# Sukikui/PTI-LDM-VAE

Hardware: AMD Instinct MI355X
Metric: vae_train_images_per_sec_256x256 (higher is better)
Workload: dtype fp16 forward operands + activations / bf16 backward operands + gradients, fp32 accumulate; 1 GPU; config/vae_dente_no_adv.json 256x256x1 batch 32/GPU: fwd + L1 + 1e-3*KL + bwd + all-reduce + Adam (perceptual term omitted: --perceptual times it; adversarial branch inactive before epoch 6, --adv times it); global_batch=32, parallelism=dp1

## Files before the change

pti_ldm_vae_amd/csrc/conv_common.h:

```cpp
#pragma once
#include "pti_common.h"

namespace pti_conv {

struct ConvArgs {
  const bf16* x;
  const unsigned char* w;
  const float* bias;
  const stat_t* in_stats;
  const float* gamma;
  const float* beta;
  const bf16* res;
  bf16* y;
  stat_t* out_stats;
  int N, H, W, Cin, Ho, Wo, Cout;
  int mode, prologue, groups, out_groups;
  float eps, inv_cnt;
  int tiles_x, tiles_y;
  int gn_mode;
  int g_groups;
  float g_inv_cnt, g_eps;
  const stat_t* g_stats; const float* g_gamma; const float* g_beta;
  float* g_sums;
  int g_T;
  bf16* act_out;
  int in_f16, res_f16, out_f16;
  int pool2;
  int relu_out;
  int w_f16;
  const bf16* x2;
  const float* p_sums;
  int x2_f16;
};
constexpr int PRO_GNB = 3;

typedef _Float16 f16x8 __attribute__((ext_vector_type(8)));
template <bool OPH>
__device__ __forceinline__ f32x16 mfma32(const bf16x8& a, const bf16x8& b, const f32x16& c) {
  if constexpr (OPH)
    return __builtin_amdgcn_mfma_f32_32x32x16_f16(__builtin_bit_cast(f16x8, a), __builtin_bit_cast(f16x8, b), c, 0, 0, 0);
  else
    return __builtin_amdgcn_mfma_f32_32x32x16_bf16(a, b, c, 0, 0, 0);
}

__host__ __device__ constexpr int pick_ck2(int cin, int ct) {
  const int ck = cin % 128 == 0 ? 128 : (cin % 64 == 0 ? 64 : 32);
  const int cap = ct >= 128 ? 128 : (ct == 64 ? 64 : 32);
  return ck < cap ? ck : cap;
}

template <int NV, int N, int O>
__device__ __forceinline__ void fold32_level(float (&v)[NV], int j) {
  if constexpr (O >= 1) {
    if constexpr (N > 1) {
      const bool hi = (j & O) != 0;
#pragma unroll
      for (int i = 0; i < N / 2; ++i) {
        const float send = hi ? v[i] : v[i + N / 2];
        const float keep = hi ? v[i + N / 2] : v[i];
        v[i] = keep + __shfl_xor(send, O, 64);
      }
    } else {
      v[0] += __shfl_xor(v[0], O, 64);
    }
    fold32_level<NV, (N > 1 ? N / 2 : 1), O / 2>(v, j);
  }
}
template <int NV>
__device__ __forceinline__ void fold32(float (&v)[NV], int j) { fold32_level<NV, NV, 16>(v, j); }

template <int KS, int CK, int CT, int PXF>
struct Cfg2 {
  static constexpr int WN = CT / 32, WM = 4 / WN;
  static constexpr int TH2 = 2 * PXF * WM, TW2 = 16;
  static constexpr int HH = TH2 + KS - 1, HW = TW2 + KS - 1;
  static constexpr int NP = HH * HW;
  static constexpr int NC = CK / 8;
  static constexpr int PIXB = CK * 2;
  static constexpr int NT = CT / 32;
  static constexpr int KPC = CK / 16;
  static constexpr int KBC = KS * KS * KPC;
  static constexpr int R = (KS == 3) ? (PXF == 2 ? 3 : 9) : KBC;
  static constexpr int WGS_PER_CU = PXF == 2 ? 4 : 2;
  static constexpr int HALO_BYTES = NP * PIXB;
  static constexpr int KEY_SHIFT = (NC == 16) ? 0 : (NC == 8 ? 1 : 2);
  static constexpr int HITERS = (NP * NC + 255) / 256;
  static constexpr int MPX = 32 * PXF * WM;
  static constexpr int EPITCH = CT * 2 + 16;
  static constexpr int EPI_BYTES = MPX * EPITCH;
  static constexpr int ENC = CT / 8;
  static constexpr int EITERS = MPX * ENC / 256;
  static constexpr int STAT_OFF = HALO_BYTES > EPI_BYTES ? HALO_BYTES : EPI_BYTES;
  static constexpr int RT_OFF = STAT_OFF + 1024 + 256;
  static constexpr int RT_BYTES = MPX * CT * 2;
  static constexpr int BIAS_OFF = RT_OFF + RT_BYTES;
  static constexpr bool GT_IN_TAIL = HALO_BYTES - EPI_BYTES >= 8 * CT;
  static constexpr int GT_OFF = GT_IN_TAIL ? EPI_BYTES : BIAS_OFF + 4 * CT;
  static constexpr int LDS_BYTES = BIAS_OFF + 4 * CT + (GT_IN_TAIL ? 0 : 8 * CT);
};


int launch_conv_ws128(const ConvArgs& a, hipStream_t st);

}
```

pti_ldm_vae_amd/csrc/conv_mfma.hip:

```cpp
#include "conv_common.h"

namespace {
using namespace pti_conv;

constexpr int TH = 8, TW = 16;

__host__ __device__ constexpr int pick_cout_tile(int cout) { return cout % 128 == 0 ? 128 : (cout % 64 == 0 ? 64 : 32); }
__host__ __device__ constexpr int pick_ck(int cin, int stride2) {
  int ck = cin % 128 == 0 ? 128 : (cin % 64 == 0 ? 64 : 32);
  return (stride2 && ck > 64) ? 64 : ck;
}
__host__ __device__ constexpr int pick_wblk(int kbc, int nt) {
  int best = 1;
  for (int w = 1; w <= kbc; ++w)
    if (kbc % w == 0 && w * nt <= 16) best = w;
  return best;
}

template <int KS, int S, int CK, int COUT_TILE>
struct Cfg {
  static constexpr int HH = (TH - 1) * S + KS, HW = (TW - 1) * S + KS;
  static constexpr int NP = HH * HW;
  static constexpr int NC = CK / 8;
  static constexpr int PIXB = CK * 2;
  static constexpr int NT = COUT_TILE / 32;
  static constexpr int KPC = CK / 16;
  static constexpr int KBC = KS * KS * KPC;
  static constexpr int WBLK = pick_wblk(KBC, NT);
  static constexpr int NSTEP = KBC / WBLK;
  static constexpr int STEPB = WBLK * NT * 1024;
  static constexpr int WM = (NT >= 2) ? 2 : 4, WN = 4 / WM;
  static constexpr int PXF = 4 / WM;
  static constexpr int CF = NT / WN;
  static constexpr int HALO_BYTES = NP * PIXB;
  static constexpr int LDS_BYTES = HALO_BYTES + 2 * STEPB;
  static constexpr int KEY_SHIFT = (NC == 16) ? 0 : (NC == 8 ? 1 : 2);
  static constexpr int WPIECES = (STEPB / 16 + 255) / 256;
  static constexpr int HITERS = (NP * NC + 255) / 256;
};

template <int KS, int S, int CK, int COUT_TILE, bool OPH>
__global__ __launch_bounds__(256, 2) void conv_mfma_kernel(ConvArgs a) {
  if (a.out_f16) fp16_saturate_on();
  using C = Cfg<KS, S, CK, COUT_TILE>;
  __shared__ __attribute__((aligned(16))) unsigned char smem[C::LDS_BYTES];
  unsigned char* halo = smem;
  unsigned char* wbuf = smem + C::HALO_BYTES;

  const int tid = threadIdx.x, lane = tid & 63, wave = tid >> 6;
  const int hsel = lane >> 5;
  int t = blockIdx.x;
  const int tile_x = t % a.tiles_x;
  t /= a.tiles_x;
  const int tile_y = t % a.tiles_y;
  const int n = t / a.tiles_y;
  const int oy0 = tile_y * TH, ox0 = tile_x * TW;
  const int ct = blockIdx.y;
  const int nchunks = a.Cin / CK;
  const int wm = wave / C::WN, wn = wave % C::WN;

  const int pad_lo = (a.mode == PTI_CONV_S2PAD) ? 0 : (a.mode == PTI_CONV_ZINS ? 2 : (KS - 1) / 2);
  const int vy0 = oy0 * S - pad_lo, vx0 = ox0 * S - pad_lo;
  const bool twox = (a.mode == PTI_CONV_UP2) || (a.mode == PTI_CONV_ZINS);
  const int VH = twox ? 2 * a.H : a.H, VW = twox ? 2 * a.W : a.W;

  int pbase[C::PXF][KS];
  int tkey[KS];
  {
    const int j = lane & 31;
    const int tx = j & 15;
#pragma unroll
    for (int kw = 0; kw < KS; ++kw) {
      const int hx = tx * S + kw;
      tkey[kw] = (hsel ^ ((hx >> C::KEY_SHIFT) & (C::NC - 1))) << 4;
#pragma unroll
      for (int i = 0; i < C::PXF; ++i) {
        const int ty = 2 * (wm * C::PXF + i) + (j >> 4);
        pbase[i][kw] = ((ty * S) * C::HW + hx) * C::PIXB;
      }
    }
  }

// ... 124 lines not shown
  const int j = lane & 31;
  stat_t* sstat = reinterpret_cast<stat_t*>(smem);
  const bool do_stats = a.out_stats != nullptr;
  const int ocpg = do_stats ? a.Cout / a.out_groups : 1;
  if (do_stats) {
    if (tid < 2 * a.out_groups) sstat[tid] = 0;
    __syncthreads();
  }
#pragma unroll
  for (int i = 0; i < C::PXF; ++i) {
    const int ty = 2 * (wm * C::PXF + i) + (j >> 4), tx = j & 15;
    const int oy = oy0 + ty, ox = ox0 + tx;
    const bool inb = (oy < a.Ho) && (ox < a.Wo);
    const size_t pix = ((size_t)(n * a.Ho + oy) * a.Wo + ox) * a.Cout;
#pragma unroll
    for (int c = 0; c < C::CF; ++c) {
#pragma unroll
      for (int q = 0; q < 4; ++q) {
        const int co = ct * COUT_TILE + (wn * C::CF + c) * 32 + 8 * q + 4 * hsel;
        float v0 = acc[i][c][4 * q + 0], v1 = acc[i][c][4 * q + 1], v2 = acc[i][c][4 * q + 2],
              v3 = acc[i][c][4 * q + 3];
        if (a.bias) {
          const f32x4 b = *(const f32x4*)(a.bias + co);
          v0 += b[0]; v1 += b[1]; v2 += b[2]; v3 += b[3];
        }
        u32x2 packed = u32x2{0u, 0u};
        if (inb) {
          if (a.res) {
            const u32x2 rr = *(const u32x2*)(a.res + pix + co);
            float e0, e1, e2, e3;
            unpack2f(rr[0], a.res_f16, e0, e1);
            unpack2f(rr[1], a.res_f16, e2, e3);
            v0 += e0; v1 += e1; v2 += e2; v3 += e3;
          }
          packed = pack4f(v0, v1, v2, v3, a.out_f16);
          *(u32x2*)(a.y + pix + co) = packed;
        }
        if (do_stats) {
          float r0, r1, r2, r3;
          unpack2f(packed[0], a.out_f16, r0, r1);
          unpack2f(packed[1], a.out_f16, r2, r3);
          if (!inb) r0 = r1 = r2 = r3 = 0.f;
          if (ocpg >= 4) {
            float s1 = (r0 + r1) + (r2 + r3), s2 = (r0 * r0 + r1 * r1) + (r2 * r2 + r3 * r3);
#pragma unroll
            for (int o = 16; o > 0; o >>= 1) {
              s1 += __shfl_xor(s1, o, 64);
              s2 += __shfl_xor(s2, o, 64);
            }
            if (j == 0) {
              const int g = co / ocpg;
              stat_add(&sstat[2 * g], s1);
              stat_add(&sstat[2 * g + 1], s2);
            }
          } else {
            float a1 = r0 + r1, a2 = r0 * r0 + r1 * r1, b1 = r2 + r3, b2 = r2 * r2 + r3 * r3;
#pragma unroll
            for (int o = 16; o > 0; o >>= 1) {
              a1 += __shfl_xor(a1, o, 64);
              a2 += __shfl_xor(a2, o, 64);
              b1 += __shfl_xor(b1, o, 64);
              b2 += __shfl_xor(b2, o, 64);
            }
            if (j == 0) {
              const int g = co / 2;
              stat_add(&sstat[2 * g], a1);
              stat_add(&sstat[2 * g + 1], a2);
              stat_add(&sstat[2 * g + 2], b1);
              stat_add(&sstat[2 * g + 3], b2);
            }
          }
        }
      }
    }
  }
  if (do_stats) {
    __syncthreads();
    const int g0 = (ct * COUT_TILE) / ocpg, ng = COUT_TILE / ocpg;
    if (tid < 2 * ng)
      atomicAdd((unsigned long long*)&a.out_stats[(n * a.out_groups + g0) * 2 + tid], (unsigned long long)sstat[2 * g0 + tid]);
  }
}

template <int KS, int CK, int CT, int PXF, bool SAVE, int FM, int PRO>
__global__ __launch_bounds__(256, (PXF == 2 ? 4 : 2)) void conv_mfma2_kernel(ConvArgs a) {
  using C = Cfg2<KS, CK, CT, PXF>;
  const int prologue = PRO >= 0 ? PRO : a.prologue;
  const bool gn_on = FM == 3 ? true : (FM == 0 ? a.gn_mode != 0 : false);
  const bool in_f16 = FM == 0 ? (bool)a.in_f16 : (FM == 1);
  const bool res_f16 = FM == 0 ? (bool)a.res_f16 : (FM == 1 || FM == 3);
  const bool out_f16 = FM == 0 ? (bool)a.out_f16 : (FM == 1);
  constexpr bool OPH = (FM == 1);
  if (out_f16) fp16_saturate_on();
  __shared__ __attribute__((aligned(16))) unsigned char smem[C::LDS_BYTES];
  unsigned char* halo = smem;
  const int tid = threadIdx.x, lane = tid & 63, wave = tid >> 6;
  const int hsel = lane >> 5;
  int t = blockIdx.x;
  const int tile_x = t % a.tiles_x;
  t /= a.tiles_x;
  const int tile_y = t % a.tiles_y;
  const int n = t / a.tiles_y;
  const int oy0 = tile_y * C::TH2, ox0 = tile_x * C::TW2;
  const int ct = blockIdx.y;
  const int nchunks = a.Cin / CK;
  const int wm = wave / C::WN, wn = wave % C::WN;

  const int pad_lo = (a.mode == PTI_CONV_ZINS) ? 2 : (KS - 1) / 2;
  const int vy0 = oy0 - pad_lo, vx0 = ox0 - pad_lo;
  const bool twox = (a.mode == PTI_CONV_UP2) || (a.mode == PTI_CONV_ZINS);
  const int VH = twox ? 2 * a.H : a.H, VW = twox ? 2 * a.W : a.W;

  int pbase[KS], tkey[KS];
  {
    const int j = lane & 31, tx = j & 15, row0 = 2 * PXF * wm + (j >> 4);
#pragma unroll
    for (int kw = 0; kw < KS; ++kw) {
      const int hx = tx + kw;
      tkey[kw] = (hsel ^ ((hx >> C::KEY_SHIFT) & (C::NC - 1))) << 4;
      pbase[kw] = (row0 * C::HW + hx) * C::PIXB;
    }
  }
  f32x16 acc[PXF];
#pragma unroll
  for (int i = 0; i < PXF; ++i)
#pragma unroll
    for (int r = 0; r < 16; ++r) acc[i][r] = 0.f;

  const int lc = tid % C::NC, lp0 = tid / C::NC;
  constexpr int PSTEP = 256 / C::NC;
  const int cpg = a.Cin / (a.groups > 0 ? a.groups : 1);
  reinterpret_cast<float*>(smem + C::STAT_OFF)[tid] = 0.f;
  float* sfl = reinterpret_cast<float*>(smem + C::STAT_OFF + 1024);
  if (prologue == PTI_PRO_GN || prologue == PTI_PRO_GN_SILU) {
    if (tid < 2 * a.groups) sfl[tid] = stat_f(a.in_stats, n * a.groups * 2 + tid);
  } else if (gn_on) {
    if (tid < 2 * a.g_groups) sfl[tid] = stat_f(a.g_stats, n * a.g_groups * 2 + tid);
  }
  float gq = 0.f, bq = 0.f;
  if (gn_on) {
    if (tid < CT) {
      gq = a.g_gamma[ct * CT + tid];
      bq = a.g_beta[ct * CT + tid];
    }
  } else if (a.bias) {
    if (tid < CT) reinterpret_cast<float*>(smem + C::BIAS_OFF)[tid] = a.bias[ct * CT + tid];
  }
  if (a.res) {
#pragma unroll
    for (int it = 0; it < C::EITERS; ++it) {
      const int slot = it * 256 + tid;
      const int p = slot / C::ENC, c = slot % C::ENC;
      const int oy = oy0 + p / C::TW2, ox = ox0 + p % C::TW2;
      if (oy < a.Ho && ox < a.Wo) {
        const bf16* src = a.res + ((size_t)(n * a.Ho + oy) * a.Wo + ox) * a.Cout + ct * CT + ((c ^ ((p >> 2) & (C::ENC - 1))) << 3);
        __builtin_amdgcn_global_load_lds((const __attribute__((address_space(1))) void*)src,
                                         (__attribute__((address_space(3))) void*)(smem + C::RT_OFF + (it * 256 + wave * 64) * 16),
                                         16, 0, 0);
      }
    }
  }

  const int epc = tid % C::ENC, epp0 = tid / C::ENC;
  constexpr int EPSTEP = 256 / C::ENC;

  for (int chunk = 0; chunk < nchunks; ++chunk) {
    const unsigned char* wlane =
        a.w + ((size_t)(ct * nchunks + chunk) * C::KBC * C::NT + wn) * 1024 + lane * 16;
    bf16x8 wa[C::R], wb[C::R];
    auto wload = [&](bf16x8 (&dst)[C::R], int g) {
#pragma unroll
      for (int u = 0; u < C::R; ++u) {
        int kb = g * C::R + u;
        kb = kb < C::KBC ? kb : C::KBC - 1;
        dst[u] = *(const bf16x8*)(wlane + (size_t)kb * C::NT * 1024);
      }
    };
    constexpr bool WLATE = (SAVE && PXF == 2) || PRO == PRO_GNB;
    if constexpr (!WLATE) wload(wa, 0);

    u32x4 raw[C::HITERS];
    u32x4 raw2[PRO == PRO_GNB ? C::HITERS : 1];
    bool ok[C::HITERS];
    {
      const __amdgpu_buffer_rsrc_t xrs = __builtin_amdgcn_make_buffer_rsrc(
          const_cast<bf16*>(a.x), 0, (unsigned)a.N * (unsigned)a.H * (unsigned)a.W * (unsigned)a.Cin * 2u, 0x00020000);
      const __amdgpu_buffer_rsrc_t x2rs = __builtin_amdgcn_make_buffer_rsrc(
          const_cast<bf16*>(PRO == PRO_GNB ? a.x2 : a.x), 0, (unsigned)a.N * (unsigned)a.H * (unsigned)a.W * (unsigned)a.Cin * 2u, 0x00020000);
      const unsigned base = ((unsigned)n * a.H * a.W * a.Cin + chunk * CK + lc * 8) * 2u;
      const unsigned rowb = (unsigned)a.W * a.Cin * 2u, pixb = (unsigned)a.Cin * 2u;
#pragma unroll
      for (int it = 0; it < C::HITERS; ++it) {
        const int p = lp0 + it * PSTEP;
        const int hy = p / C::HW, hx = p - hy * C::HW;
        const int vy = vy0 + hy, vx = vx0 + hx;
        bool v = (p < C::NP) && (unsigned)vy < (unsigned)VH && (unsigned)vx < (unsigned)VW;
        int iy = vy, ix = vx;
        if (twox) {
          if (a.mode == PTI_CONV_ZINS) v = v && !((vy | vx) & 1);
          iy = vy >> 1;
          ix = vx >> 1;
        }
        ok[it] = v;
        const unsigned off = v ? base + (unsigned)iy * rowb + (unsigned)ix * pixb : 0x80000000u;
        raw[it] = __builtin_bit_cast(u32x4, __builtin_amdgcn_raw_buffer_load_b128(xrs, off, 0, 0));
        if constexpr (PRO == PRO_GNB) raw2[it] = __builtin_bit_cast(u32x4, __builtin_amdgcn_raw_buffer_load_b128(x2rs, off, 0, 0));
      }
    }
    if (chunk == 0) __syncthreads();
    float sc[8], sh[8];
    [[maybe_unused]] float gnb_b = 0.f, gnb_d = 0.f;
    if constexpr (PRO == PRO_GNB) {
      const int ch0 = chunk * CK + lc * 8, g = ch0 / cpg;
      const float mean = stat_f(a.in_stats, (n * a.groups + g) * 2) * a.inv_cnt;
      const float rstd = rsqrtf(fmaxf(stat_f(a.in_stats, (n * a.groups + g) * 2 + 1) * a.inv_cnt - mean * mean, 0.f) + a.eps);
      float t1 = 0.f, t2 = 0.f;
      for (int cc = g * cpg; cc < (g + 1) * cpg; ++cc) {
        const f32x2 sv = *(const f32x2*)(a.p_sums + ((size_t)n * a.Cin + cc) * 2);
        const float gm = a.gamma[cc];
        t1 += gm * sv[0];
        t2 += gm * sv[1];
      }
      const float c1 = t1 * a.inv_cnt, c2 = t2 * a.inv_cnt;
#pragma unroll
      for (int j = 0; j < 8; ++j) sc[j] = rstd * a.gamma[ch0 + j];
      gnb_b = -rstd * rstd * c2;
      gnb_d = -rstd * c1 - gnb_b * mean;
    } else if (prologue != PTI_PRO_NONE) {
      float mu_[8], rs_[8];
      gn_params<8>(sfl, a.gamma, a.beta, chunk * CK + lc * 8, cpg, a.inv_cnt, a.eps, sc, sh, mu_, rs_);
    }
    if (chunk > 0) __syncthreads();
#pragma unroll
    for (int it = 0; it < C::HITERS; ++it) {
      const int p = lp0 + it * PSTEP;
      if (p < C::NP) {
        const int hy = p / C::HW, hx = p - hy * C::HW;
        u32x4 r = raw[it];
        if constexpr (PRO == PRO_GNB) {
          if (ok[it]) {
            float f[8], h[8];
            unpack8(r, f);
            unpack8f(raw2[it], h, a.x2_f16 != 0);
#pragma unroll
            for (int j = 0; j < 8; ++j) f[j] = fmaf(sc[j], f[j], fmaf(gnb_b, h[j], gnb_d));
            r = pack8(f);
          }
        } else if (prologue != PTI_PRO_NONE && ok[it]) {
          float f[8];
          unpack8f(r, f, in_f16);
          if (PXF == 4 && prologue == PTI_PRO_GN_SILU) {
#pragma unroll
            for (int j = 0; j < 8; j += 2) {
              const f32x2 o = gn_silu2(f32x2{f[j], f[j + 1]}, f32x2{sc[j], sc[j + 1]}, f32x2{sh[j], sh[j + 1]});
              f[j] = o[0];
              f[j + 1] = o[1];
            }
          } else {
#pragma unroll
            for (int j = 0; j < 8; ++j) {
              float v = f[j] * sc[j] + sh[j];
              if (prologue == PTI_PRO_GN_SILU) v = silu_f(v);
              f[j] = v;
            }
          }
          r = OPH ? pack8f(f, true) : pack8(f);
        } else if (in_f16 && !OPH) {
          float f[8];
          unpack8f(r, f, true);
          r = pack8(f);
        }
        const int key = (hx >> C::KEY_SHIFT) & (C::NC - 1);
        *(u32x4*)(halo + p * C::PIXB + ((lc ^ key) << 4)) = r;
      }
    }
    __syncthreads();

    if constexpr (SAVE) {
      if (ct == 0) {
        constexpr int PL = (KS - 1) / 2;
        constexpr int SITERS = C::TH2 * C::TW2 * C::NC / 256;
        const __amdgpu_buffer_rsrc_t srs = __builtin_amdgcn_make_buffer_rsrc(
            a.act_out, 0, (unsigned)a.N * (unsigned)a.H * (unsigned)a.W * (unsigned)a.Cin * 2u, 0x00020000);
#pragma unroll 1
        for (int it = 0; it < SITERS; ++it) {
          const int idx = tid + it * 256;
          const int c8 = idx % C::NC, pi = idx / C::NC;
          const int hy = pi / C::TW2 + PL, hx = pi % C::TW2 + PL;
          const int vy = vy0 + hy, vx = vx0 + hx;
          if (vy < a.H && vx < a.W) {
            const int key = (hx >> C::KEY_SHIFT) & (C::NC - 1);
            u32x4 piece = *(const u32x4*)(halo + (hy * C::HW + hx) * C::PIXB + ((c8 ^ key) << 4));
            if constexpr (OPH) {
              float f[8];
              unpack8f(piece, f, true);
              piece = pack8(f);
            }
            __builtin_amdgcn_raw_buffer_store_b128(__builtin_bit_cast(bu32x4, piece), srs,
                                                   ((unsigned)((n * a.H + vy) * a.W + vx) * a.Cin + chunk * CK + c8 * 8) * 2u, 0, 2 );
          }
        }
      }
    }

    if constexpr (WLATE) wload(wa, 0);
    const int txl = lane & 15;
    auto baddr = [&](int kb) -> const unsigned char* {
      kb = kb < C::KBC ? kb : C::KBC - 1;
      const int tap = kb / C::KPC, kc = kb - tap * C::KPC;
      const int kh = (KS == 3) ? tap / 3 : 0, kw = tap - kh * KS;
      const int hx = txl + kw;
      const int tk = (hsel ^ ((hx >> C::KEY_SHIFT) & (C::NC - 1))) << 4;
      return halo + pbase[0] + (kh * C::HW + kw) * C::PIXB + ((kc * 32) ^ tk);
    };
    bf16x8 b0[PXF], b1[PXF];
    auto bread = [&](bf16x8 (&dst)[PXF], int kb) {
      const unsigned char* bp = baddr(kb);
#pragma unroll
      for (int i = 0; i < PXF; ++i) dst[i] = *(const bf16x8*)(bp + 2 * i * C::HW * C::PIXB);
    };
    auto group = [&](const bf16x8 (&w)[C::R], int g) {
      const int kb0 = g * C::R;
#pragma unroll
      for (int u = 0; u < C::R; ++u) {
        if ((u & 1) == 0) {
          bread(b1, kb0 + u + 1);
#pragma unroll
          for (int i = 0; i < PXF; ++i) acc[i] = mfma32<OPH>(w[u], b0[i], acc[i]);
        } else {
          bread(b0, kb0 + u + 1);
#pragma unroll
          for (int i = 0; i < PXF; ++i) acc[i] = mfma32<OPH>(w[u], b1[i], acc[i]);
        }
      }
      if (C::R & 1) {
#pragma unroll
        for (int i = 0; i < PXF; ++i) b0[i] = b1[i];
      }
    };
    constexpr int NG = C::KBC / C::R;
    bread(b0, 0);
    if constexpr (NG == 1) {
      group(wa, 0);
    } else {
#pragma clang loop unroll(disable)
      for (int g = 0; g < NG; g += 2) {
        wload(wb, g + 1);
        group(wa, g);
        wload(wa, g + 2);
        group(wb, g + 1);
      }
    }
  }

  const int j = lane & 31;
  unsigned char* etile = smem;
  const bool do_stats = (FM == 2 || FM == 3) ? false : a.out_stats != nullptr;
  const int ocpg = do_stats ? a.Cout / a.out_groups : 1;
  __syncthreads();
  float* gtab = reinterpret_cast<float*>(smem + C::GT_OFF);
  if (gn_on) {
    if (tid < CT) {
      gtab[tid] = gq;
      gtab[CT + tid] = bq;
    }
    __syncthreads();
  }
  const unsigned char* rtile = smem + C::RT_OFF;
  const int col0 = wn * 32 + 4 * hsel;
  float st1[4] = {0.f, 0.f, 0.f, 0.f}, st2[4] = {0.f, 0.f, 0.f, 0.f};
  float su1[4] = {0.f, 0.f, 0.f, 0.f}, su2[4] = {0.f, 0.f, 0.f, 0.f};
  if (gn_on) {
    const int gcpg = a.Cout / a.g_groups;
    float* gsm = reinterpret_cast<float*>(smem + C::STAT_OFF);
    float L[32];
#pragma unroll
    for (int q = 0; q < 4; ++q) {
      const int col = col0 + 8 * q, ch0 = ct * CT + col;
      float scv[4], shv[4], muv[4], rsv[4], l1[4] = {0.f, 0.f, 0.f, 0.f}, l2[4] = {0.f, 0.f, 0.f, 0.f};
      gn_params<4>(sfl, gtab - ct * CT, gtab + CT - ct * CT, ch0, gcpg, a.g_inv_cnt, a.g_eps, scv, shv, muv, rsv);
      float nmr[4];
#pragma unroll
      for (int r = 0; r < 4; ++r) nmr[r] = -muv[r] * rsv[r];
#pragma unroll
      for (int i = 0; i < PXF; ++i) {
        const int p = (2 * PXF * wm + 2 * i + (j >> 4)) * 16 + (j & 15);
        const bool inb = (oy0 + (p >> 4) < a.Ho) && (ox0 + (p & 15) < a.Wo);
        unsigned char* ep = etile + p * C::EPITCH + col * 2;
        const u32x2 rr = *(const u32x2*)(rtile + p * (CT * 2) + ((((col >> 3) ^ (p >> 2)) & (C::ENC - 1)) << 4) + (col & 7) * 2);
        float xv[4];
        unpack2f(rr[0], res_f16, xv[0], xv[1]);
        unpack2f(rr[1], res_f16, xv[2], xv[3]);
        float dv[4];
#pragma unroll
        for (int r = 0; r < 4; ++r) {
          float v = acc[i][4 * q + r];
          if (a.gn_mode == 2) v *= dsilu_f(xv[r] * scv[r] + shv[r]);
          dv[r] = v;
        }
        const u32x2 packed = pack4(dv[0], dv[1], dv[2], dv[3]);
        *(u32x2*)ep = packed;
        if (inb) {
#pragma unroll
          for (int r = 0; r < 4; ++r) {
            l1[r] += dv[r];
            l2[r] = fmaf(dv[r], fmaf(xv[r], rsv[r], nmr[r]), l2[r]);
          }
        }
      }
#pragma unroll
      for (int r = 0; r < 4; ++r) {
        L[8 * q + 2 * r] = l1[r];
        L[8 * q + 2 * r + 1] = l2[r];
      }
    }
    fold32<32>(L, j);
    gsm[wm * 2 * CT + col0 * 2 + 16 * (j >> 3) + (j & 7)] = L[0];
  } else {
#pragma unroll
  for (int i = 0; i < PXF; ++i) {
    const int p = (2 * PXF * wm + 2 * i + (j >> 4)) * 16 + (j & 15);
    const bool inb = (oy0 + (p >> 4) < a.Ho) && (ox0 + (p & 15) < a.Wo);
#pragma unroll
    for (int q = 0; q < 4; ++q) {
      const int col = col0 + 8 * q;
      float v0 = acc[i][4 * q + 0], v1 = acc[i][4 * q + 1], v2 = acc[i][4 * q + 2], v3 = acc[i][4 * q + 3];
      if (a.bias) {
        const f32x4 b = *(const f32x4*)(smem + C::BIAS_OFF + col * 4);
        v0 += b[0]; v1 += b[1]; v2 += b[2]; v3 += b[3];
      }
      unsigned char* ep = etile + p * C::EPITCH + col * 2;
      if (a.res) {
        const u32x2 rr = *(const u32x2*)(rtile + p * (CT * 2) + ((((col >> 3) ^ (p >> 2)) & (C::ENC - 1)) << 4) + (col & 7) * 2);
        float e0, e1, e2, e3;
        unpack2f(rr[0], res_f16, e0, e1);
        unpack2f(rr[1], res_f16, e2, e3);
        v0 += e0; v1 += e1; v2 += e2; v3 += e3;
      }
      if constexpr (FM == 1 && PRO == PTI_PRO_NONE) {
        if (a.relu_out) { v0 = fmaxf(v0, 0.f); v1 = fmaxf(v1, 0.f); v2 = fmaxf(v2, 0.f); v3 = fmaxf(v3, 0.f); }
      }
      const u32x2 packed = pack4f(v0, v1, v2, v3, out_f16);
      *(u32x2*)ep = packed;
      if (do_stats && inb) {
        float r0, r1, r2, r3;
        unpack2f(packed[0], out_f16, r0, r1);
        unpack2f(packed[1], out_f16, r2, r3);
        if (ocpg >= 4) {
          st1[q] += (r0 + r1) + (r2 + r3);
          st2[q] += (r0 * r0 + r1 * r1) + (r2 * r2 + r3 * r3);
        } else {
          st1[q] += r0 + r1; st2[q] += r0 * r0 + r1 * r1;
          su1[q] += r2 + r3; su2[q] += r2 * r2 + r3 * r3;
        }
      }
    }
  }
  }
  if (do_stats) {
    stat_t* sstat = reinterpret_cast<stat_t*>(smem + C::STAT_OFF);
    if (ocpg >= 4) {
      float v[8];
#pragma unroll
      for (int q = 0; q < 4; ++q) { v[2 * q] = st1[q]; v[2 * q + 1] = st2[q]; }
      fold32<8>(v, j);
      if ((j & 3) == 0) {
        const int idx = j >> 2, q = idx >> 1;
        const int g = (ct * CT + col0 + 8 * q) / ocpg;
        stat_add(&sstat[2 * g + (idx & 1)], v[0]);
      }
    } else {
      float v[16];
#pragma unroll
      for (int q = 0; q < 4; ++q) { v[4 * q] = st1[q]; v[4 * q + 1] = st2[q]; v[4 * q + 2] = su1[q]; v[4 * q + 3] = su2[q]; }
      fold32<16>(v, j);
      if ((j & 1) == 0) {
        const int idx = j >> 1, q = idx >> 2;
        const int g = (ct * CT + col0 + 8 * q) / 2;
        stat_add(&sstat[2 * g + (idx & 3)], v[0]);
      }
    }
  }
  __syncthreads();
  const __amdgpu_buffer_rsrc_t yrs = __builtin_amdgcn_make_buffer_rsrc(
      a.y, 0, ((unsigned)a.N * (unsigned)a.Ho * (unsigned)a.Wo * (unsigned)a.Cout * 2u) >> (a.pool2 ? 2 : 0), 0x00020000);
  if ((FM == 0 || FM == 2) && a.pool2) {
    constexpr int PITERS = (C::EITERS + 3) / 4;
#pragma unroll
    for (int it = 0; it < PITERS; ++it) {
      const int idx = tid + it * 256;
      const int c8 = idx % C::ENC, pp = idx / C::ENC;
      const int py = pp / 8, px = pp % 8;
      const int oy = (oy0 >> 1) + py, ox = (ox0 >> 1) + px;
      if (pp < C::MPX / 4 && oy < (a.Ho >> 1) && ox < (a.Wo >> 1)) {
        const unsigned char* src = etile + ((2 * py) * 16 + 2 * px) * C::EPITCH + c8 * 16;
        float s_[8], f_[8];
        unpack8f(*(const u32x4*)src, s_, out_f16);
        unpack8f(*(const u32x4*)(src + C::EPITCH), f_, out_f16);
#pragma unroll
        for (int q = 0; q < 8; ++q) s_[q] += f_[q];
        unpack8f(*(const u32x4*)(src + 16 * C::EPITCH), f_, out_f16);
#pragma unroll
        for (int q = 0; q < 8; ++q) s_[q] += f_[q];
        unpack8f(*(const u32x4*)(src + 17 * C::EPITCH), f_, out_f16);
#pragma unroll
        for (int q = 0; q < 8; ++q) s_[q] += f_[q];
        __builtin_amdgcn_raw_buffer_store_b128(__builtin_bit_cast(bu32x4, pack8f(s_, out_f16)), yrs,
                                               ((unsigned)((n * (a.Ho >> 1) + oy) * (a.Wo >> 1) + ox) * a.Cout + ct * CT + c8 * 8) * 2u, 0, 2);
      }
    }
  } else
#pragma unroll
  for (int it = 0; it < C::EITERS; ++it) {
    const int p = epp0 + it * EPSTEP;
    const int oy = oy0 + (p >> 4), ox = ox0 + (p & 15);
    if (oy < a.Ho && ox < a.Wo)
      __builtin_amdgcn_raw_buffer_store_b128(__builtin_bit_cast(bu32x4, *(const u32x4*)(etile + p * C::EPITCH + epc * 16)), yrs,
                                             ((unsigned)((n * a.Ho + oy) * a.Wo + ox) * a.Cout + ct * CT + epc * 8) * 2u, 0, 2);
  }
  if (gn_on) {
    if (tid < 2 * CT) {
      const float* gsm = reinterpret_cast<const float*>(smem + C::STAT_OFF);
      float v = gsm[tid];
#pragma unroll
      for (int m = 1; m < C::WM; ++m) v += gsm[m * 2 * CT + tid];
      a.g_sums[(((size_t)n * a.g_T + tile_y * a.tiles_x + tile_x) * a.Cout + ct * CT) * 2 + tid] = v;
    }
  } else if (do_stats) {
    const stat_t* sstat = reinterpret_cast<const stat_t*>(smem + C::STAT_OFF);
    const int g0 = (ct * CT) / ocpg, ng = CT / ocpg;
    if (tid < 2 * ng)
      atomicAdd((unsigned long long*)&a.out_stats[(n * a.out_groups + g0) * 2 + tid], (unsigned long long)sstat[2 * g0 + tid]);
  }
}

template <int KS, int CK, int CT, int PXF>
int launch2_cfg(ConvArgs a, hipStream_t st) {
  using C = Cfg2<KS, CK, CT, PXF>;
  a.tiles_x = cdiv(a.Wo, C::TW2);
  a.tiles_y = cdiv(a.Ho, C::TH2);
  a.g_T = a.tiles_x * a.tiles_y;
  dim3 grid(a.N * a.tiles_x * a.tiles_y, a.Cout / CT);
  const bool res = a.res != nullptr;
  const int fm = (a.w_f16 && a.in_f16 && a.out_f16 && (a.res_f16 || !res)) ? 1
               : (!a.in_f16 && !a.out_f16 && (!a.res_f16 || !res)) ? 2
               : (!a.in_f16 && !a.out_f16 && a.res_f16) ? 3 : 0;
  const bool fwd_silu = fm == 1 && a.prologue == PTI_PRO_GN_SILU && !a.gn_mode && !a.pool2;
  const bool fwd_plain = fm == 1 && a.prologue == PTI_PRO_NONE && !a.gn_mode && !a.pool2;
  const bool dgrad = fm == 2 && a.prologue == PTI_PRO_NONE && !a.gn_mode && !a.out_stats;
  const bool dgrad_gn = fm == 3 && a.prologue == PTI_PRO_NONE && a.gn_mode && !a.out_stats && !a.pool2;
  if (a.x2) {
    if constexpr (KS == 3 && PXF == 4 && CT == 128) {
      if (!(fm == 3 && a.gn_mode && a.act_out && !a.out_stats && !a.pool2 && a.mode == PTI_CONV_S1 && !a.relu_out)) return 4;
      PTI_LAUNCH((conv_mfma2_kernel<KS, CK, CT, PXF, true, 3, PRO_GNB>), grid, dim3(256), 0, st, a);
      return 0;
    } else {
      return 4;
    }
// ... 348 lines not shown
```

Before: 2735 images/s.

## Specialize narrow 3x3 conv kernel with incremental addressing and DPP reductions

For the PXF=2, 3x3, fixed-format conv variants, this adds a NARROW specialization. Halo, residual and saved-activation address generation moves to strength-reduced incremental offsets, and whole waves with no work skip the halo-load iterations. The GroupNorm backward epilogue is rewritten with precomputed per-quad parameters and a pinned dSiLU. The cross-lane stat folds now use DPP, ds_swizzle and permlane16_swap instead of generic shuffles. The aim is to cut integer ALU, LDS-shuffle and register cost in the hot conv kernel, at the cost of more code paths and a possible change in numerical ordering.

```diff
diff --git a/pti_ldm_vae_amd/csrc/conv_common.h b/pti_ldm_vae_amd/csrc/conv_common.h
--- a/pti_ldm_vae_amd/csrc/conv_common.h
+++ b/pti_ldm_vae_amd/csrc/conv_common.h
@@ -69,6 +69,43 @@
 template <int NV>
 __device__ __forceinline__ void fold32(float (&v)[NV], int j) { fold32_level<NV, NV, 16>(v, j); }
 
+template <int O>
+__device__ __forceinline__ float xor_lane(float v) {
+  static_assert(O == 8 || O == 4 || O == 2 || O == 1, "xor distance inside a 16-lane row");
+  const unsigned u = __float_as_uint(v);
+  if constexpr (O == 8) return __uint_as_float(__builtin_amdgcn_update_dpp(0u, u, 0x128 , 0xf, 0xf, false));
+  else if constexpr (O == 4) return __uint_as_float(__builtin_amdgcn_ds_swizzle(u, 0x101f ));
+  else if constexpr (O == 2) return __uint_as_float(__builtin_amdgcn_update_dpp(0u, u, 0x4e , 0xf, 0xf, false));
+  else return __uint_as_float(__builtin_amdgcn_update_dpp(0u, u, 0xb1 , 0xf, 0xf, false));
+}
+template <int NV, int N, int O>
+__device__ __forceinline__ void fold32x_level(float (&v)[NV], int j) {
+  if constexpr (O >= 1) {
+    if constexpr (N > 1 && O == 16) {
+#pragma unroll
+      for (int i = 0; i < N / 2; ++i) {
+        const auto sw = __builtin_amdgcn_permlane16_swap(__float_as_uint(v[i]), __float_as_uint(v[i + N / 2]), false, false);
+        v[i] = __uint_as_float(sw[0]) + __uint_as_float(sw[1]);
+      }
+    } else if constexpr (N > 1) {
+      const bool hi = (j & O) != 0;
+#pragma unroll
+      for (int i = 0; i < N / 2; ++i) {
+        const float send = hi ? v[i] : v[i + N / 2];
+        const float keep = hi ? v[i + N / 2] : v[i];
+        v[i] = keep + xor_lane<O>(send);
+      }
+    } else if constexpr (O == 16) {
+      v[0] += __shfl_xor(v[0], 16, 64);
+    } else {
+      v[0] += xor_lane<O>(v[0]);
+    }
+    fold32x_level<NV, (N > 1 ? N / 2 : 1), O / 2>(v, j);
+  }
+}
+template <int NV>
+__device__ __forceinline__ void fold32x(float (&v)[NV], int j) { fold32x_level<NV, NV, 16>(v, j); }
+
 template <int KS, int CK, int CT, int PXF>
 struct Cfg2 {
   static constexpr int WN = CT / 32, WM = 4 / WN;
diff --git a/pti_ldm_vae_amd/csrc/conv_mfma.hip b/pti_ldm_vae_amd/csrc/conv_mfma.hip
--- a/pti_ldm_vae_amd/csrc/conv_mfma.hip
+++ b/pti_ldm_vae_amd/csrc/conv_mfma.hip
@@ -1,3 +1,5 @@
+#include <type_traits>
+
 #include "conv_common.h"
 
 namespace {
@@ -288,6 +290,78 @@
   }
 }
 
+__device__ __forceinline__ f32x2 dsilu_times2(f32x2 acc, f32x2 v) {
+#pragma clang fp contract(off)
+#pragma clang fp reassociate(off)
+  const f32x2 t = v * -1.4426950408889634f;
+  f32x2 s;
+  s[0] = __builtin_amdgcn_rcpf(1.0f + __builtin_amdgcn_exp2f(t[0]));
+  s[1] = __builtin_amdgcn_rcpf(1.0f + __builtin_amdgcn_exp2f(t[1]));
+  const f32x2 sa = s * acc;
+  f32x2 b = (1.0f - s) * v;
+  asm("" : "+v"(b));
+  return sa * (1.0f + b);
+}
+
+__device__ __forceinline__ void gn_quad_pinned(const float* sfl, const float* gam, const float* bet, int ch0, int cpg,
+                                               float inv_cnt, float eps, float* sc, float* sh, float* rs, float* nmr) {
+#pragma clang fp contract(off)
+#pragma clang fp reassociate(off)
+  const bool pow2 = (cpg & (cpg - 1)) == 0;
+  const f32x4 gm = *(const f32x4*)gam, bt = *(const f32x4*)bet;
+  auto rstd_fused = [&](const f32x2 st, float& mean) {
+    mean = st[0] * inv_cnt;
+    const float t = st[1] * inv_cnt;
+    return __builtin_amdgcn_rsqf(fmaxf(__builtin_fmaf(-mean, mean, t), 0.f) + eps);
+  };
+  if (pow2 && cpg >= 4) {
+    float mean;
+    const float rstd = rstd_fused(*(const f32x2*)(sfl + 2 * (ch0 >> __builtin_ctz(cpg))), mean);
+    const float nm = rstd * -mean;
+#pragma unroll
+    for (int r = 0; r < 4; ++r) {
+      sc[r] = rstd * gm[r];
+      sh[r] = __builtin_fmaf(nm, gm[r], bt[r]);
+      rs[r] = rstd;
+      nmr[r] = nm;
+    }
+  } else if (cpg == 2) {
+#pragma unroll
+    for (int k = 0; k < 2; ++k) {
+      float mean;
+      const float rstd = rstd_fused(*(const f32x2*)(sfl + 2 * ((ch0 >> 1) + k)), mean);
+      const float rm = rstd * mean;
+#pragma unroll
+      for (int r = 2 * k; r < 2 * k + 2; ++r) {
+        sc[r] = rstd * gm[r];
+        sh[r] = __builtin_fmaf(-rm, gm[r], bt[r]);
+        rs[r] = rstd;
+        nmr[r] = -rm;
+      }
+    }
+  } else {
+#pragma unroll
+    for (int r = 0; r < 4; ++r) {
+      const int g = cpg == 1 ? ch0 + r : (ch0 + r) / cpg;
+      const f32x2 st = *(const f32x2*)(sfl + 2 * g);
+      const float mean = st[0] * inv_cnt;
+      float t = st[1] * inv_cnt, var;
+      if (r < 2) {
+        float mm = mean * mean;
+        asm("" : "+v"(t), "+v"(mm));
+        var = t - mm;
+      } else {
+        var = __builtin_fmaf(-mean, mean, t);
+      }
+      const float rstd = __builtin_amdgcn_rsqf(fmaxf(var, 0.f) + eps);
+      sc[r] = rstd * gm[r];
+      sh[r] = __builtin_fmaf(-sc[r], mean, bt[r]);
+      rs[r] = rstd;
+      nmr[r] = -mean * rstd;
+    }
+  }
+}
+
 template <int KS, int CK, int CT, int PXF, bool SAVE, int FM, int PRO>
 __global__ __launch_bounds__(256, (PXF == 2 ? 4 : 2)) void conv_mfma2_kernel(ConvArgs a) {
   using C = Cfg2<KS, CK, CT, PXF>;
@@ -297,6 +371,7 @@
   const bool res_f16 = FM == 0 ? (bool)a.res_f16 : (FM == 1 || FM == 3);
   const bool out_f16 = FM == 0 ? (bool)a.out_f16 : (FM == 1);
   constexpr bool OPH = (FM == 1);
+  constexpr bool NARROW = PXF == 2 && KS == 3 && FM != 0;
   if (out_f16) fp16_saturate_on();
   __shared__ __attribute__((aligned(16))) unsigned char smem[C::LDS_BYTES];
   unsigned char* halo = smem;
@@ -335,6 +410,14 @@
 
   const int lc = tid % C::NC, lp0 = tid / C::NC;
   constexpr int PSTEP = 256 / C::NC;
+  const int wpiece0 = __builtin_amdgcn_readfirstlane(tid & ~63);
+  auto wave_has_piece = [&](int it) { return it * 256 + 255 < C::NP * C::NC || it * 256 + wpiece0 < C::NP * C::NC; };
+  constexpr int HDY = PSTEP / C::HW, HDX = PSTEP % C::HW;
+  auto halo_step = [](int& hy, int& hx) {
+    hx += HDX;
+    hy += HDY;
+    if (hx >= C::HW) { hx -= C::HW; ++hy; }
+  };
   const int cpg = a.Cin / (a.groups > 0 ? a.groups : 1);
   reinterpret_cast<float*>(smem + C::STAT_OFF)[tid] = 0.f;
   float* sfl = reinterpret_cast<float*>(smem + C::STAT_OFF + 1024);
@@ -352,23 +435,43 @@
   } else if (a.bias) {
     if (tid < CT) reinterpret_cast<float*>(smem + C::BIAS_OFF)[tid] = a.bias[ct * CT + tid];
   }
+  constexpr int EPSTEP = 256 / C::ENC;
   if (a.res) {
-#pragma unroll
-    for (int it = 0; it < C::EITERS; ++it) {
-      const int slot = it * 256 + tid;
-      const int p = slot / C::ENC, c = slot % C::ENC;
-      const int oy = oy0 + p / C::TW2, ox = ox0 + p % C::TW2;
-      if (oy < a.Ho && ox < a.Wo) {
-        const bf16* src = a.res + ((size_t)(n * a.Ho + oy) * a.Wo + ox) * a.Cout + ct * CT + ((c ^ ((p >> 2) & (C::ENC - 1))) << 3);
-        __builtin_amdgcn_global_load_lds((const __attribute__((address_space(1))) void*)src,
-                                         (__attribute__((address_space(3))) void*)(smem + C::RT_OFF + (it * 256 + wave * 64) * 16),
-                                         16, 0, 0);
+    if constexpr (NARROW) {
+      const unsigned char* rsrc = reinterpret_cast<const unsigned char*>(a.res) + ((size_t)n * a.Ho * a.Wo * a.Cout + ct * CT) * 2;
+      const int rc = tid % C::ENC, rp0 = tid / C::ENC;
+      const int ry = oy0 + (rp0 >> 4), rx = ox0 + (rp0 & 15);
+      const unsigned rstep = (unsigned)(EPSTEP >> 4) * a.Wo * a.Cout * 2u;
+      unsigned roff = (unsigned)(ry * a.Wo + rx) * a.Cout * 2u;
+      const bool rxin = rx < a.Wo;
+#pragma unroll
+      for (int it = 0; it < C::EITERS; ++it) {
+        const int p = rp0 + it * EPSTEP;
+        if (rxin && ry + it * (EPSTEP >> 4) < a.Ho) {
+          const unsigned char* src = rsrc + (roff + (unsigned)((rc ^ ((p >> 2) & (C::ENC - 1))) << 4));
+          __builtin_amdgcn_global_load_lds((const __attribute__((address_space(1))) void*)src,
+                                           (__attribute__((address_space(3))) void*)(smem + C::RT_OFF + (it * 256 + wave * 64) * 16),
+                                           16, 0, 0);
+        }
+        roff += rstep;
+      }
+    } else {
+#pragma unroll
+      for (int it = 0; it < C::EITERS; ++it) {
+        const int slot = it * 256 + tid;
+        const int p = slot / C::ENC, c = slot % C::ENC;
+        const int oy = oy0 + p / C::TW2, ox = ox0 + p % C::TW2;
+        if (oy < a.Ho && ox < a.Wo) {
+          const bf16* src = a.res + ((size_t)(n * a.Ho + oy) * a.Wo + ox) * a.Cout + ct * CT + ((c ^ ((p >> 2) & (C::ENC - 1))) << 3);
+          __builtin_amdgcn_global_load_lds((const __attribute__((address_space(1))) void*)src,
+                                           (__attribute__((address_space(3))) void*)(smem + C::RT_OFF + (it * 256 + wave * 64) * 16),
+                                           16, 0, 0);
+        }
       }
     }
   }
 
   const int epc = tid % C::ENC, epp0 = tid / C::ENC;
-  constexpr int EPSTEP = 256 / C::ENC;
 
   for (int chunk = 0; chunk < nchunks; ++chunk) {
     const unsigned char* wlane =
@@ -395,22 +498,41 @@
           const_cast<bf16*>(PRO == PRO_GNB ? a.x2 : a.x), 0, (unsigned)a.N * (unsigned)a.H * (unsigned)a.W * (unsigned)a.Cin * 2u, 0x00020000);
       const unsigned base = ((unsigned)n * a.H * a.W * a.Cin + chunk * CK + lc * 8) * 2u;
       const unsigned rowb = (unsigned)a.W * a.Cin * 2u, pixb = (unsigned)a.Cin * 2u;
-#pragma unroll
-      for (int it = 0; it < C::HITERS; ++it) {
-        const int p = lp0 + it * PSTEP;
-        const int hy = p / C::HW, hx = p - hy * C::HW;
-        const int vy = vy0 + hy, vx = vx0 + hx;
-        bool v = (p < C::NP) && (unsigned)vy < (unsigned)VH && (unsigned)vx < (unsigned)VW;
-        int iy = vy, ix = vx;
-        if (twox) {
-          if (a.mode == PTI_CONV_ZINS) v = v && !((vy | vx) & 1);
-          iy = vy >> 1;
-          ix = vx >> 1;
-        }
-        ok[it] = v;
-        const unsigned off = v ? base + (unsigned)iy * rowb + (unsigned)ix * pixb : 0x80000000u;
-        raw[it] = __builtin_bit_cast(u32x4, __builtin_amdgcn_raw_buffer_load_b128(xrs, off, 0, 0));
-        if constexpr (PRO == PRO_GNB) raw2[it] = __builtin_bit_cast(u32x4, __builtin_amdgcn_raw_buffer_load_b128(x2rs, off, 0, 0));
+      if constexpr (NARROW) {
+        int hy = lp0 / C::HW, hx = lp0 - hy * C::HW;
+        const int tsh = twox ? 1 : 0, zmask = (a.mode == PTI_CONV_ZINS) ? 1 : 0;
+#pragma unroll
+        for (int it = 0; it < C::HITERS; ++it) {
+          raw[it] = u32x4{0u, 0u, 0u, 0u};
+          ok[it] = false;
+          if (wave_has_piece(it)) {
+            const int vy = vy0 + hy, vx = vx0 + hx;
+            const bool v = (hy < C::HH) && (unsigned)vy < (unsigned)VH && (unsigned)vx < (unsigned)VW && !((vy | vx) & zmask);
+            ok[it] = v;
+            const unsigned off = v ? base + (unsigned)(vy >> tsh) * rowb + (unsigned)(vx >> tsh) * pixb : 0x80000000u;
+            raw[it] = __builtin_bit_cast(u32x4, __builtin_amdgcn_raw_buffer_load_b128(xrs, off, 0, 0));
+            if constexpr (PRO == PRO_GNB) raw2[it] = __builtin_bit_cast(u32x4, __builtin_amdgcn_raw_buffer_load_b128(x2rs, off, 0, 0));
+          }
+          halo_step(hy, hx);
+        }
+      } else {
+#pragma unroll
+        for (int it = 0; it < C::HITERS; ++it) {
+          const int p = lp0 + it * PSTEP;
+          const int hy = p / C::HW, hx = p - hy * C::HW;
+          const int vy = vy0 + hy, vx = vx0 + hx;
+          bool v = (p < C::NP) && (unsigned)vy < (unsigned)VH && (unsigned)vx < (unsigned)VW;
+          int iy = vy, ix = vx;
+          if (twox) {
+            if (a.mode == PTI_CONV_ZINS) v = v && !((vy | vx) & 1);
+            iy = vy >> 1;
+            ix = vx >> 1;
+          }
+          ok[it] = v;
+          const unsigned off = v ? base + (unsigned)iy * rowb + (unsigned)ix * pixb : 0x80000000u;
+          raw[it] = __builtin_bit_cast(u32x4, __builtin_amdgcn_raw_buffer_load_b128(xrs, off, 0, 0));
+          if constexpr (PRO == PRO_GNB) raw2[it] = __builtin_bit_cast(u32x4, __builtin_amdgcn_raw_buffer_load_b128(x2rs, off, 0, 0));
+        }
       }
     }
     if (chunk == 0) __syncthreads();
@@ -437,11 +559,23 @@
       gn_params<8>(sfl, a.gamma, a.beta, chunk * CK + lc * 8, cpg, a.inv_cnt, a.eps, sc, sh, mu_, rs_);
     }
     if (chunk > 0) __syncthreads();
+    [[maybe_unused]] int shy = 0, shx = 0;
+    if constexpr (NARROW) {
+      shy = lp0 / C::HW;
+      shx = lp0 - shy * C::HW;
+    }
 #pragma unroll
     for (int it = 0; it < C::HITERS; ++it) {
       const int p = lp0 + it * PSTEP;
-      if (p < C::NP) {
-        const int hy = p / C::HW, hx = p - hy * C::HW;
+      if constexpr (NARROW) {
+        if (!wave_has_piece(it)) continue;
+      }
+      if (NARROW ? shy < C::HH : p < C::NP) {
+        int hx = shx;
+        if constexpr (!NARROW) {
+          const int hy = p / C::HW;
+          hx = p - hy * C::HW;
+        }
         u32x4 r = raw[it];
         if constexpr (PRO == PRO_GNB) {
           if (ok[it]) {
@@ -479,6 +613,7 @@
         const int key = (hx >> C::KEY_SHIFT) & (C::NC - 1);
         *(u32x4*)(halo + p * C::PIXB + ((lc ^ key) << 4)) = r;
       }
+      if constexpr (NARROW) halo_step(shy, shx);
     }
     __syncthreads();
 
@@ -488,22 +623,47 @@
         constexpr int SITERS = C::TH2 * C::TW2 * C::NC / 256;
         const __amdgpu_buffer_rsrc_t srs = __builtin_amdgcn_make_buffer_rsrc(
             a.act_out, 0, (unsigned)a.N * (unsigned)a.H * (unsigned)a.W * (unsigned)a.Cin * 2u, 0x00020000);
+        if constexpr (NARROW) {
+          const int hx = (lp0 & 15) + PL, vx = vx0 + hx;
+          int vy = vy0 + (lp0 >> 4) + PL;
+          const int key = (hx >> C::KEY_SHIFT) & (C::NC - 1);
+          const unsigned char* sp = halo + (((lp0 >> 4) + PL) * C::HW + hx) * C::PIXB + ((lc ^ key) << 4);
+          unsigned soff = ((unsigned)((n * a.H + vy) * a.W + vx) * a.Cin + chunk * CK + lc * 8) * 2u;
+          const unsigned sstep = (unsigned)(PSTEP >> 4) * a.W * a.Cin * 2u;
+          const bool vxin = vx < a.W;
 #pragma unroll 1
-        for (int it = 0; it < SITERS; ++it) {
-          const int idx = tid + it * 256;
-          const int c8 = idx % C::NC, pi = idx / C::NC;
-          const int hy = pi / C::TW2 + PL, hx = pi % C::TW2 + PL;
-          const int vy = vy0 + hy, vx = vx0 + hx;
-          if (vy < a.H && vx < a.W) {
-            const int key = (hx >> C::KEY_SHIFT) & (C::NC - 1);
-            u32x4 piece = *(const u32x4*)(halo + (hy * C::HW + hx) * C::PIXB + ((c8 ^ key) << 4));
-            if constexpr (OPH) {
-              float f[8];
-              unpack8f(piece, f, true);
-              piece = pack8(f);
+          for (int it = 0; it < SITERS; ++it) {
+            if (vxin && vy < a.H) {
+              u32x4 piece = *(const u32x4*)sp;
+              if constexpr (OPH) {
+                float f[8];
+                unpack8f(piece, f, true);
+                piece = pack8(f);
+              }
+              __builtin_amdgcn_raw_buffer_store_b128(__builtin_bit_cast(bu32x4, piece), srs, soff, 0, 2 );
             }
-            __builtin_amdgcn_raw_buffer_store_b128(__builtin_bit_cast(bu32x4, piece), srs,
-                                                   ((unsigned)((n * a.H + vy) * a.W + vx) * a.Cin + chunk * CK + c8 * 8) * 2u, 0, 2 );
+            vy += PSTEP >> 4;
+            sp += (PSTEP >> 4) * C::HW * C::PIXB;
+            soff += sstep;
+          }
+        } else {
+#pragma unroll 1
+          for (int it = 0; it < SITERS; ++it) {
+            const int idx = tid + it * 256;
+            const int c8 = idx % C::NC, pi = idx / C::NC;
+            const int hy = pi / C::TW2 + PL, hx = pi % C::TW2 + PL;
+            const int vy = vy0 + hy, vx = vx0 + hx;
+            if (vy < a.H && vx < a.W) {
+              const int key = (hx >> C::KEY_SHIFT) & (C::NC - 1);
+              u32x4 piece = *(const u32x4*)(halo + (hy * C::HW + hx) * C::PIXB + ((c8 ^ key) << 4));
+              if constexpr (OPH) {
+                float f[8];
+                unpack8f(piece, f, true);
+                piece = pack8(f);
+              }
+              __builtin_amdgcn_raw_buffer_store_b128(__builtin_bit_cast(bu32x4, piece), srs,
+                                                     ((unsigned)((n * a.H + vy) * a.W + vx) * a.Cin + chunk * CK + c8 * 8) * 2u, 0, 2 );
+            }
           }
         }
       }
@@ -576,7 +736,57 @@
   const int col0 = wn * 32 + 4 * hsel;
   float st1[4] = {0.f, 0.f, 0.f, 0.f}, st2[4] = {0.f, 0.f, 0.f, 0.f};
   float su1[4] = {0.f, 0.f, 0.f, 0.f}, su2[4] = {0.f, 0.f, 0.f, 0.f};
-  if (gn_on) {
+  const int p0 = (2 * PXF * wm + (j >> 4)) * 16 + (j & 15);
+  const int eoff = p0 * C::EPITCH + col0 * 2;
+  const int roff0 = p0 * (CT * 2) + hsel * 8;
+  const int rkey = (((4 * wn) ^ (p0 >> 2)) & (C::ENC - 1)) << 4;
+  if (gn_on && NARROW) {
+    const int gcpg = a.Cout / a.g_groups;
+    float* gsm = reinterpret_cast<float*>(smem + C::STAT_OFF);
+    float L[32];
+    bool inb[PXF];
+#pragma unroll
+    for (int i = 0; i < PXF; ++i) inb[i] = (oy0 + (p0 >> 4) + 2 * i < a.Ho) && (ox0 + (p0 & 15) < a.Wo);
+#pragma unroll
+    for (int q = 0; q < 4; ++q) {
+      float scv[4], shv[4], rsv[4], nmr[4], l1[4] = {0.f, 0.f, 0.f, 0.f}, l2[4] = {0.f, 0.f, 0.f, 0.f};
+      gn_quad_pinned(sfl, gtab + col0 + 8 * q, gtab + CT + col0 + 8 * q, ct * CT + col0 + 8 * q, gcpg, a.g_inv_cnt, a.g_eps,
+                     scv, shv, rsv, nmr);
+      auto quad = [&](auto silu) {
+#pragma unroll
+        for (int i = 0; i < PXF; ++i) {
+          const u32x2 rr = *(const u32x2*)(rtile + roff0 + i * 32 * (CT * 2) + (rkey ^ (((q ^ (8 * i)) & (C::ENC - 1)) << 4)));
+          float xv[4], dv[4];
+          unpack2f(rr[0], res_f16, xv[0], xv[1]);
+          unpack2f(rr[1], res_f16, xv[2], xv[3]);
+#pragma unroll
+          for (int r = 0; r < 4; r += 2) {
+            f32x2 d2 = f32x2{acc[i][4 * q + r], acc[i][4 * q + r + 1]};
+            if constexpr (decltype(silu)::value)
+              d2 = dsilu_times2(d2, f32x2{fmaf(xv[r], scv[r], shv[r]), fmaf(xv[r + 1], scv[r + 1], shv[r + 1])});
+            dv[r] = d2[0];
+            dv[r + 1] = d2[1];
+          }
+          *(u32x2*)(etile + eoff + i * 32 * C::EPITCH + q * 16) = pack4(dv[0], dv[1], dv[2], dv[3]);
+          if (inb[i]) {
+#pragma unroll
+            for (int r = 0; r < 4; ++r) {
+              l1[r] += dv[r];
+              l2[r] = fmaf(dv[r], fmaf(xv[r], rsv[r], nmr[r]), l2[r]);
+            }
+          }
+        }
+      };
+      if (a.gn_mode == 2) quad(std::true_type{}); else quad(std::false_type{});
+#pragma unroll
+      for (int r = 0; r < 4; ++r) {
+        L[8 * q + 2 * r] = l1[r];
+        L[8 * q + 2 * r + 1] = l2[r];
+      }
+    }
+    fold32x<32>(L, j);
+    gsm[wm * 2 * CT + col0 * 2 + 16 * (j >> 3) + (j & 7)] = L[0];
+  } else if (gn_on) {
     const int gcpg = a.Cout / a.g_groups;
     float* gsm = reinterpret_cast<float*>(smem + C::STAT_OFF);
     float L[32];
@@ -635,9 +845,11 @@
         const f32x4 b = *(const f32x4*)(smem + C::BIAS_OFF + col * 4);
         v0 += b[0]; v1 += b[1]; v2 += b[2]; v3 += b[3];
       }
-      unsigned char* ep = etile + p * C::EPITCH + col * 2;
+      unsigned char* ep = NARROW ? etile + eoff + i * 32 * C::EPITCH + q * 16 : etile + p * C::EPITCH + col * 2;
       if (a.res) {
-        const u32x2 rr = *(const u32x2*)(rtile + p * (CT * 2) + ((((col >> 3) ^ (p >> 2)) & (C::ENC - 1)) << 4) + (col & 7) * 2);
+        const unsigned char* rp = NARROW ? rtile + roff0 + i * 32 * (CT * 2) + (rkey ^ (((q ^ (8 * i)) & (C::ENC - 1)) << 4))
+                                         : rtile + p * (CT * 2) + ((((col >> 3) ^ (p >> 2)) & (C::ENC - 1)) << 4) + (col & 7) * 2;
+        const u32x2 rr = *(const u32x2*)rp;
         float e0, e1, e2, e3;
         unpack2f(rr[0], res_f16, e0, e1);
         unpack2f(rr[1], res_f16, e2, e3);
@@ -669,7 +881,7 @@
       float v[8];
 #pragma unroll
       for (int q = 0; q < 4; ++q) { v[2 * q] = st1[q]; v[2 * q + 1] = st2[q]; }
-      fold32<8>(v, j);
+      if constexpr (NARROW) fold32x<8>(v, j); else fold32<8>(v, j);
       if ((j & 3) == 0) {
         const int idx = j >> 2, q = idx >> 1;
         const int g = (ct * CT + col0 + 8 * q) / ocpg;
@@ -679,7 +891,7 @@
       float v[16];
 #pragma unroll
       for (int q = 0; q < 4; ++q) { v[4 * q] = st1[q]; v[4 * q + 1] = st2[q]; v[4 * q + 2] = su1[q]; v[4 * q + 3] = su2[q]; }
-      fold32<16>(v, j);
+      if constexpr (NARROW) fold32x<16>(v, j); else fold32<16>(v, j);
       if ((j & 1) == 0) {
         const int idx = j >> 1, q = idx >> 2;
         const int g = (ct * CT + col0 + 8 * q) / 2;
```

Result: no change. 2753 images/s (median of 6 runs) (+0.7%).
